# qdrant/qdrant

Measured on AMD Instinct MI355X. Metric: QPS @ recall@10, brute-force, d=768 10M vecs, f32 cosine top-10, higher is better.
Workload: dtype f32 (int8 prefilter + exact f32 re-score)

## Files before the change

### qdrant_amd/csrc/api_core.hip

```cpp
#include "api_internal.hpp"

namespace qmx {

static thread_local std::string g_last_error;
const std::string &last_error_text() { return g_last_error; }

void set_error(const char *fmt, ...) {
    char buf[1024];
    va_list ap;
    va_start(ap, fmt);
    vsnprintf(buf, sizeof(buf), fmt, ap);
    va_end(ap);
    g_last_error = buf;
}

int32_t hip_status(hipError_t e, const char *what, const char *file, int line) {
    set_error("HIP error %d (%s) at %s:%d: %s", (int)e, hipGetErrorString(e), file, line, what);
    (void)hipGetLastError();
    switch (e) {
        case hipErrorOutOfMemory: return QMX_ERR_OUT_OF_MEMORY;
        case hipErrorNoDevice:
        case hipErrorInvalidDevice:
        case hipErrorNoBinaryForGpu:
        case hipErrorInsufficientDriver: return QMX_ERR_NO_DEVICE;
        case hipErrorNotReady: return QMX_ERR_NOT_READY;
        case hipErrorInvalidValue: return QMX_ERR_BAD_ARG;
        default: return QMX_ERR_OTHER;
    }
}

static const char *const g_option_names[OPT_COUNT] = {"no_mfma_scan", "no_mfma16", "no_prescan", "prescan_shift", "hnsw_log_cap", "no_split_scan", "split_min_queries", "no_split256", "no_pq_pair", "no_pq_prefilter", "pq_prefilter_min_queries", "hnsw_pq_per_cu", "tq_rotate_block", "no_topk_small", "verify_max_per_query", "hnsw_pq_direct_walk", "hnsw_pq_table_build", "hnsw_no_pq_prefilter", "hnsw_no_lds_visited", "pq_lut_no_lds", "hnsw_per_cu", "hnsw_reference_heap_order", "tq_wide_min_queries", "tq_wide_high_digit", "sq_wide_min_queries", "i8_resident", "debug"};
struct OptionTable {
    std::atomic<int64_t> v[OPT_COUNT];
    int64_t initial[OPT_COUNT];
    OptionTable() {
        for (int i = 0; i < OPT_COUNT; ++i) {
            char env[64] = "QMX_";
            size_t k = 4;
            for (const char *c = g_option_names[i]; *c && k + 1 < sizeof(env); ++c) env[k++] = (char)toupper((unsigned char)*c);
            env[k] = 0;
            const char *e = getenv(env);
            int64_t val = 0;
            if (e) { val = (*e >= '0' && *e <= '9') ? atoll(e) : 1; }
            if (i == OPT_PRESCAN_SHIFT && !e) val = 10;
            if (i == OPT_SPLIT_MIN_QUERIES && !e) val = 1;
            if (i == OPT_PQ_PREFILTER_MIN_QUERIES && !e) val = 4;
            if (i == OPT_TQ_WIDE_MIN_QUERIES && !e) val = 33;
            if (i == OPT_SQ_WIDE_MIN_QUERIES && !e) val = 33;
            if (i == OPT_I8_RESIDENT && !e) val = 1;
            initial[i] = val;
            v[i].store(val, std::memory_order_relaxed);
        }
    }
};
static OptionTable g_options;
int64_t option(Option o) { return g_options.v[o].load(std::memory_order_relaxed); }

static thread_local const void *g_last_kernel = nullptr;
const void *last_noted_kernel() { return g_last_kernel; }
void note_kernel(const void *host_function) { g_last_kernel = host_function; }

void clear_stale_error() {
    hipError_t e = hipGetLastError();
    if (e != hipSuccess) {
// ... 98 lines not shown
```

### qdrant_amd/csrc/api_search.hip

```cpp
#include "api_internal.hpp"

extern "C" {



static int32_t split_stage(qmx_query *q, const char *what) {
    if (option(OPT_DEBUG) < 2) return QMX_OK;
    hipError_t e = hipStreamSynchronize(q->stream);
    fprintf(stderr, "[qmx] split stage %-28s %s\n", what, e == hipSuccess ? "ok" : hipGetErrorString(e));
    fflush(stderr);
    return e == hipSuccess ? QMX_OK : QMX_ERR_OTHER;
}

static int32_t verify_pool(qmx_query *q, unsigned char *plan, VerifyPool *vp) {
    const uint32_t cap = (uint32_t)std::min<uint64_t>(std::max<uint64_t>((uint64_t)q->nq * SPLIT_VCAP, 262144), 1u << 26);
    QMX_TRY(q->sp_ver.reserve(((size_t)cap * 2 + (size_t)q->nq * 2) * 4));
    QMX_TRY(q->sp_vscores.reserve((size_t)cap * 4));
    uint32_t *b = (uint32_t *)q->sp_ver.p;
    vp->ids = b;
    vp->qsel = b + cap;
    vp->off = b + (size_t)2 * cap;
    vp->cnt = vp->off + q->nq;
    vp->used = (uint32_t *)(plan + 24);
    vp->cap = cap;
// ... 334 lines not shown
            QMX_TRY(q->sp_probe.reserve((size_t)q->nq * (split_i8_probe() + 1) * 4));
            QMX_TRY(q->sp_pscores.reserve((size_t)q->nq * split_i8_probe() * 4));
        }
        plan = (unsigned char *)q->sp_plan.p;
        float *f = (float *)q->sp_f32.p;
        sp_qnorm = f; sp_thr = f + 256; sp_band = f + 512; sp_scales = f + 768; sp_qmax = f + 1024;
        const int sshift = (int)std::min<int64_t>(std::max<int64_t>(option(OPT_PRESCAN_SHIFT) + (s->d_rows_split ? 1 : -2), 1), 20);
        const uint64_t S = std::min<uint64_t>(n_cand, std::max<uint64_t>(n_cand >> sshift, 8192));
        if (q->sp_sample_n != S || q->sp_sample_of != n_cand) {
            QMX_TRY(q->sp_sample.reserve((size_t)S * 4));
            ::qmx::clear_stale_error();
            hipLaunchKernelGGL(sample_ids_kernel, dim3((uint32_t)((S + 255) / 256)), dim3(256), 0, q->stream, (uint32_t *)q->sp_sample.p, (uint32_t)S, n_cand / S);
            QMX_HIP(hipGetLastError());
            q->sp_sample_n = S;
            q->sp_sample_of = n_cand;
        }
        QMX_HIP(hipMemsetAsync(plan, 0, pl.zero_bytes, q->stream));
    }
    for (uint32_t tile0 = 0; tile0 < q->nq; tile0 += TQ) {
        const uint32_t nq_tile = std::min<uint32_t>(TQ, q->nq - tile0);
        if (split && (nq_tile > MAX_QT_TOPK || s->d_rows_split)) {
            if (is_stopped && *is_stopped) {
                set_error("search cancelled");
                return QMX_ERR_CANCELLED;
            }
            const uint32_t S = (uint32_t)q->sp_sample_n;
            const uint32_t *d_sample = (const uint32_t *)q->sp_sample.p;
            uint64_t *gthr = (uint64_t *)q->gthr.p + tile0;
            ScanArgs a;
            fill_args(q, tile0, nq_tile, a);
            a.n_cand = n_cand;
            a.top = top;
            QMX_TRY(q->scores.reserve((size_t)nq_tile * S * sizeof(float)));
            QMX_TRY(score_matrix_enqueue(q, tile0, nq_tile, d_sample, S, (float *)q->scores.p, S, nullptr));
            QMX_TRY(launch_custom_topk(q->stream, (const float *)q->scores.p, S, d_sample, a.del, nq_tile, top, d_out + (size_t)tile0 * top, d_counts + tile0, gthr));
            QMX_TRY(split_stage(q, "prescan"));
            if (s->split_i8) {
                float *sp_texact = sp_qnorm, *sp_qscale = sp_qmax;
                QMX_TRY(launch_split_i8_pack(q->stream, (const float *)q->enc.p + (size_t)tile0 * s->dim, nq_tile, s->dim, s->d_i8_scale, gthr, s->d_i8_stats,
                                             s->row_norm_max, q->sp_bq.p, sp_qscale, sp_band, sp_thr, sp_texact, (uint32_t *)q->sp_cnt.p, SPLIT_QT_MAX));
                QMX_TRY(split_stage(q, "int8 pack"));
                const uint32_t np = split_i8_probe();
                uint32_t *probe_ids = (uint32_t *)q->sp_probe.p, *probe_cnt = probe_ids + (size_t)q->nq * np;
                int *tile_ovf = (int *)(plan + pl.tile_ovf) + split_tiles.size();
                const uint32_t sstride = 16;
                for (uint32_t ph = 1; ph <= 2; ++ph) {
                    const uint32_t phase = ph | (sstride << 8);
                    size_t slot = 0;
                    if (timed) QMX_TRY(timing_begin(q, &slot));
                    QMX_TRY(launch_scan_i8copy(q->stream, a, q->sp_bq.p, sp_qscale, sp_thr, s->num_cus, s->d_rows_split, q->sp_wl.p, phase));
                    q->last_kernel = last_noted_kernel();
                    if (timed) QMX_TRY(timing_end(q, slot));
                    QMX_TRY(launch_split_regroup(q->stream, a, q->sp_wl.p, s->num_cus, (uint64_t *)q->sp_cand.p, (uint32_t *)q->sp_cnt.p, SPLIT_CAND_CAP, tile_ovf,
                                                 phase, SPLIT_QT));
                    QMX_TRY(launch_split_i8_probe(q->stream, (const uint64_t *)q->sp_cand.p, (const uint32_t *)q->sp_cnt.p, SPLIT_CAND_CAP, sp_band, nq_tile, top, tile_ovf,
                                                  probe_ids + (size_t)tile0 * np, probe_cnt + tile0));
                    const void *scan_kernel = q->last_kernel;
                    PairSel psel{nullptr, np, probe_cnt};
                    QMX_TRY(score_pairs_device(q, psel, probe_ids, (uint64_t)(tile0 + nq_tile) * np, (float *)q->sp_pscores.p, false));
                    q->last_kernel = scan_kernel;
                    QMX_TRY(launch_split_i8_bound(q->stream, (const float *)q->sp_pscores.p + (size_t)tile0 * np, probe_cnt + tile0, nq_tile, top, sp_band, sp_qscale,
                                                  sp_thr, sp_texact));
                }
                QMX_TRY(split_stage(q, "int8 scan"));
                QMX_TRY(launch_split_select(q->stream, (const uint64_t *)q->sp_cand.p, (const uint32_t *)q->sp_cnt.p, SPLIT_CAND_CAP, sp_band, nq_tile, top, vp, tile0,
                                            tile_ovf, (uint32_t *)(plan + pl.ovf_q) + tile0, (SplitStats *)plan, sp_texact));
                QMX_TRY(split_stage(q, "select"));
                split_tiles.push_back({tile0, nq_tile});
// ... 363 lines not shown
```

### qdrant_amd/csrc/common.hpp

```cpp
#pragma once
#include <hip/hip_runtime.h>
#include <hip/hip_fp16.h>
#include <stdint.h>
#include <atomic>
#include <string>

#include "../../include/qdrant_amd.h"

namespace qmx {

void set_error(const char *fmt, ...);
int32_t hip_status(hipError_t e, const char *what, const char *file, int line);
void clear_stale_error();

enum Option {
    OPT_NO_MFMA_SCAN = 0,
    OPT_NO_MFMA16,
    OPT_NO_PRESCAN,
    OPT_PRESCAN_SHIFT,
    OPT_HNSW_LOG_CAP,
    OPT_NO_SPLIT_SCAN,
    OPT_SPLIT_MIN_QUERIES,
    OPT_NO_SPLIT256,
    OPT_NO_PQ_PAIR,
    OPT_NO_PQ_PREFILTER,
    OPT_PQ_PREFILTER_MIN_QUERIES,
    OPT_HNSW_PQ_PER_CU,
    OPT_TQ_ROTATE_BLOCK,
    OPT_NO_TOPK_SMALL,
    OPT_VERIFY_MAX_PER_QUERY,
    OPT_HNSW_PQ_DIRECT_WALK,
    OPT_HNSW_PQ_TABLE_BUILD,
    OPT_HNSW_NO_PQ_PREFILTER,
    OPT_HNSW_NO_LDS_VISITED,
    OPT_PQ_LUT_NO_LDS,
    OPT_HNSW_PER_CU,
    OPT_HNSW_REFERENCE_HEAP_ORDER,
    OPT_TQ_WIDE_MIN_QUERIES,
    OPT_TQ_WIDE_HIGH_DIGIT,
    OPT_SQ_WIDE_MIN_QUERIES,
    OPT_I8_RESIDENT,
    OPT_DEBUG,
    OPT_COUNT
};
int64_t option(Option o);
struct DeviceOnce {
    std::atomic<uint64_t> done{0};
    int dev = 0;
    bool need() {
        if (hipGetDevice(&dev) != hipSuccess) { dev = 0; return true; }
        return dev >= 64 || !(done.load(std::memory_order_acquire) & (1ull << dev));
    }
    void mark() { if (dev < 64) done.fetch_or(1ull << dev, std::memory_order_release); }
};
void note_kernel(const void *host_function);
#define QMX_NOTE_KERNEL(fn) ::qmx::note_kernel(reinterpret_cast<const void *>(fn))

#define QMX_HIP(expr)                                                        \
    do {                                                                     \
        hipError_t e__ = (expr);                                             \
        if (e__ != hipSuccess) return ::qmx::hip_status(e__, #expr, __FILE__, __LINE__); \
    } while (0)

#define QMX_TRY(expr)                           \
    do {                                        \
        int32_t s__ = (expr);                   \
        if (s__ != QMX_OK) return s__;          \
    } while (0)

#define QMX_REQUIRE(cond, code, ...)            \
    do {                                        \
        if (!(cond)) {                          \
            ::qmx::set_error(__VA_ARGS__);      \
            return (code);                      \
// ... 89 lines not shown
```

### qdrant_amd/csrc/custom_query.hip

```cpp
#include "custom_combine.hpp"
#include "kernels.hpp"

namespace qmx {

__device__ __forceinline__ float custom_combine(const qmx_custom_query &q, const float *sims, uint64_t stride, const float *coefs) {
    const float *s = sims + (uint64_t)q.first * stride;
    return custom_score_by(q.kind, q.n_a, q.n_b, coefs + q.coef_first, [&](uint32_t e) { return s[(uint64_t)e * stride]; });
}

__global__ __launch_bounds__(256) void custom_combine_kernel(const qmx_custom_query *queries, uint32_t n_queries, const float *sims, uint64_t n,
                                                             const float *coefs, float *out) {
    const uint64_t c = (uint64_t)blockIdx.x * 256 + threadIdx.x;
    const uint32_t qi = blockIdx.y;
    if (c >= n || qi >= n_queries) return;
    out[(uint64_t)qi * n + c] = custom_combine(queries[qi], sims + c, n, coefs);
}

int32_t launch_custom_combine(hipStream_t st, const qmx_custom_query *d_queries, uint32_t n_queries, const float *d_sims, uint64_t n,
                              const float *d_coefs, float *d_out) {
    if (n == 0 || n_queries == 0) return QMX_OK;
    ::qmx::clear_stale_error();
    hipLaunchKernelGGL(custom_combine_kernel, dim3((uint32_t)((n + 255) / 256), n_queries), dim3(256), 0, st, d_queries, n_queries, d_sims, n, d_coefs, d_out);
    QMX_HIP(hipGetLastError());
    return QMX_OK;
// ... 201 lines not shown
            if (k != 0 && k >= t) surv[atomicAdd(&sh_cnt, 1u)] = k;
        }
        __syncthreads();
        const uint32_t cnt = sh_cnt;
        for (uint32_t i = threadIdx.x; i < cnt; i += CT_BLOCK) {
            const uint64_t my = surv[i];
            uint32_t r = 0;
            for (uint32_t j = 0; j < cnt; ++j) r += (surv[j] > my || (surv[j] == my && j < i)) ? 1u : 0u;
            if (r < ptop) {
                qmx_scored_point p;
                p.idx = key_idx(my);
                p.score = key_score(my);
                out[(uint64_t)q * top + off + r] = p;
                if (r == ptop - 1) sh_bound = my;
            }
        }
        const uint32_t found = cnt < ptop ? cnt : ptop;
        for (uint32_t i = found + threadIdx.x; i < ptop; i += CT_BLOCK) out[(uint64_t)q * top + off + i] = qmx_scored_point{0u, 0.0f};
        total += found;
        __syncthreads();
        bound = sh_bound;
        if (bound == 0) {
            for (uint32_t i = off + WAVE + threadIdx.x; i < top; i += CT_BLOCK) out[(uint64_t)q * top + i] = qmx_scored_point{0u, 0.0f};
            break;
        }
        __syncthreads();
    }
    if (threadIdx.x == 0) {
        out_counts[q] = total;
        if (bound_out) bound_out[q] = total == top ? bound : 0ull;
    }
}

int32_t launch_custom_topk(hipStream_t st, const float *d_scores, uint64_t n, const uint32_t *d_ids, const DeletedView &del, uint32_t n_queries,
                           uint32_t top, qmx_scored_point *d_out, uint32_t *d_counts, uint64_t *d_bound) {
    if (n_queries == 0) return QMX_OK;
    ::qmx::clear_stale_error();
    if (n >= 1 && n <= CTS_MAX_N && !option(OPT_NO_TOPK_SMALL)) {
        static thread_local DeviceOnce attr_once;
        if (attr_once.need()) {
            QMX_HIP(hipFuncSetAttribute(reinterpret_cast<const void *>(custom_topk_small_kernel), hipFuncAttributeMaxDynamicSharedMemorySize, (int)(CTS_MAX_N * 8)));
            attr_once.mark();
        }
        hipLaunchKernelGGL(custom_topk_small_kernel, dim3(n_queries), dim3(CT_BLOCK), (size_t)n * 8, st, d_scores, (uint32_t)n, d_ids, del, top, d_out, d_counts, d_bound);
        QMX_HIP(hipGetLastError());
        return QMX_OK;
    }
    hipLaunchKernelGGL(custom_topk_kernel, dim3(n_queries), dim3(CT_BLOCK), 0, st, d_scores, n, d_ids, del, top, d_out, d_counts, d_bound);
    QMX_HIP(hipGetLastError());
    return QMX_OK;
}

}
```

### qdrant_amd/csrc/kernels.hpp

```cpp
#pragma once
#include "common.hpp"

namespace qmx {

constexpr int MAX_QT = 16;
constexpr int SCAN_BLOCK = 512;
constexpr int MAX_TOP_FAST = 64;

struct TqEc {
    const int16_t *weights;
    const float *xm;
    float weight_scale, mm_const;
};
struct ScanArgs {
    const void *rows;
    uint64_t n_rows;
    uint64_t row_stride;
    uint32_t dim;
    uint32_t nseg;
    uint32_t rem_pieces;
    uint32_t tail_start;
    uint32_t aux_off;
    uint32_t nq;
    const void *queries;
// ... 186 lines not shown
    uint32_t *vis_log;
    uint32_t log_cap;
    uint32_t *sel_ids;
    float *sel_scores;
    uint32_t *sel_cnt;
    uint32_t *lock;
    uint32_t lds_query_bytes;
    uint32_t row_bytes;
    const unsigned char *batch_queries;
    uint64_t batch_q_stride;
    uint32_t *next;
};
int32_t launch_hnsw_build_bq(hipStream_t st, const ScanArgs &a, const HnswBuildArgs &h, int phase, uint32_t grid, int *per_cu);
int32_t launch_hnsw_build_sq(hipStream_t st, int distance, const ScanArgs &a, const HnswBuildArgs &h, int phase, uint32_t grid, int *per_cu);
int32_t launch_hnsw_build_dense(hipStream_t st, int dtype, int distance, const ScanArgs &a, const HnswBuildArgs &h, int phase,
                                uint32_t grid, int *per_cu);
int32_t launch_hnsw_build_maxsim_dense(hipStream_t st, int dtype, int distance, const ScanArgs &a, const HnswBuildArgs &h, int phase, uint32_t grid,
                                       int *per_cu);
int32_t launch_hnsw_build_maxsim_sq(hipStream_t st, int distance, const ScanArgs &a, const HnswBuildArgs &h, int phase, uint32_t grid, int *per_cu);
int32_t launch_hnsw_build_maxsim_bq(hipStream_t st, const ScanArgs &a, const HnswBuildArgs &h, int phase, uint32_t grid, int *per_cu);
int32_t launch_hnsw_build_tq(hipStream_t st, const ScanArgs &a, const HnswBuildArgs &h, int phase, uint32_t grid, int *per_cu);
int32_t launch_hnsw_build_tq_l1(hipStream_t st, const ScanArgs &a, const HnswBuildArgs &h, int phase, uint32_t grid, int *per_cu, uint32_t rot_dim,
                                uint32_t padded_dim);
int32_t launch_hnsw_build_pq(hipStream_t st, const ScanArgs &a, const HnswBuildArgs &h, int phase, uint32_t grid, int *per_cu);
int32_t launch_hnsw_build_maxsim_pq(hipStream_t st, const ScanArgs &a, const HnswBuildArgs &h, int phase, uint32_t grid, int *per_cu);
int32_t launch_hnsw_build_maxsim_tq(hipStream_t st, const ScanArgs &a, const HnswBuildArgs &h, int phase, uint32_t grid, int *per_cu);
int32_t launch_pq_pair_table(hipStream_t st, uint32_t distance, uint32_t dim, const qmx_pq_params &pq, const float *d_centroids, float *d_pair);
int32_t launch_u8_row_norms(hipStream_t st, const void *rows, uint64_t row_stride, uint64_t n, uint32_t dim, uint32_t flags, float *norms_f, int32_t *norms_i);
constexpr uint32_t HNSW_LDS_QUERY_MAX = 150 * 1024;

int32_t launch_scan_dense(hipStream_t st, int dtype, int distance, int qt, ScanMode mode,
                          const ScanArgs &a, int num_cus, uint32_t *grid_out);
int32_t launch_scan_f32_mfma(hipStream_t st, int qt, ScanMode mode, const ScanArgs &a, int num_cus, uint32_t *grid_out);
bool sq_mfma_ok(uint32_t distance, uint32_t actual_dim);
int32_t launch_scan_sq_mfma(hipStream_t st, int qt, ScanMode mode, const ScanArgs &a, int num_cus, uint32_t *grid_out);
int32_t launch_scan_f16_mfma(hipStream_t st, int qt, ScanMode mode, const ScanArgs &a, int num_cus, uint32_t *grid_out);
struct PairSel {
    const uint32_t *qsel;
    uint32_t per_query;
    const uint32_t *counts;
    const uint32_t *limit;
    __device__ __forceinline__ uint32_t query_of(uint64_t item) const {
        if (qsel) return qsel[item];
        if (per_query) return (uint32_t)(item / per_query);
        return (uint32_t)item;
    }
    __device__ __forceinline__ bool live(uint64_t item, uint32_t qi) const {
        if (limit && item >= (uint64_t)*limit) return false;
        if (per_query && counts) return (uint32_t)(item % per_query) < counts[qi];
        return true;
    }
};

int32_t launch_pairs_dense(hipStream_t st, int dtype, int distance, const ScanArgs &a, const PairSel &sel,
                           uint64_t n_items, int num_cus);
int32_t launch_pairs_sq(hipStream_t st, int distance, const ScanArgs &a, const PairSel &sel, uint64_t n_items, int num_cus);
int32_t launch_scan_sq(hipStream_t st, int distance, int qt, ScanMode mode, const ScanArgs &a, int num_cus,
                       uint32_t *grid_out);
int32_t launch_sq_encode(hipStream_t st, int distance, const qmx_sq_params &sp, uint32_t dim, const float *in, uint64_t n,
                         uint8_t *codes_out, uint64_t codes_stride, float *offsets_out, uint8_t *rows_out, int is_query,
                         uint32_t aux_off);
int32_t launch_sq_split(hipStream_t st, const void *rows, uint64_t row_stride, uint64_t n, uint32_t actual_dim, void *codes,
                        float *offsets);
int32_t launch_sq_gather_rows(hipStream_t st, const void *codes, const float *offsets, uint32_t actual_dim, const uint32_t *ids,
                              uint32_t n, uint64_t n_rows, void *rows_out, int *err_flag);
int32_t launch_sq_internal_query(hipStream_t st, const void *codes, const float *offsets, uint32_t actual_dim, const uint32_t *ids,
// ... 19 lines not shown
size_t pq_prefilter_table_bytes(uint32_t m, uint32_t nq);
uint32_t pq_prefilter_grid(int num_cus, uint32_t nq, uint32_t *n_slabs_out);
size_t pq_prefilter_wlists_counts_bytes(uint32_t grid);
size_t pq_prefilter_wlists_bytes(uint32_t grid, uint32_t wcap);
int32_t launch_pq_lut8(hipStream_t st, const void *d_luts, uint32_t q_stride, uint32_t nq, uint32_t m, uint32_t ncent, const uint64_t *d_gthr, void *d_table8,
                       int32_t *d_thr, float *d_band);
int32_t launch_pq_prefilter(hipStream_t st, const ScanArgs &a, const void *d_rot, const void *d_table8, const int32_t *d_thr, uint32_t nq, int num_cus,
                            void *d_wlists, uint32_t wcap, uint32_t *grid_out);
int32_t launch_split_refine(hipStream_t st, const uint64_t *d_cand, const uint32_t *d_cand_cnt, uint32_t cap, const float *d_band, uint32_t nq, uint32_t top,
                            const float *d_scales, float *d_thr);
size_t split_wlists_bytes(int num_cus);
int32_t launch_split_regroup(hipStream_t st, const ScanArgs &a, const void *d_wlists, int num_cus, uint64_t *d_cand, uint32_t *d_cand_cnt, uint32_t cap,
                             int *d_overflow, uint32_t phase, uint32_t qt);
size_t split_copy_bytes(uint64_t n, uint32_t dim, int half);
int32_t launch_split_copy(hipStream_t st, const void *rows, uint64_t row_stride, uint64_t n, uint32_t dim, float row_scale, void *d_out, int half);
struct SplitStats {
    unsigned long long candidates;
    unsigned long long verified;
    uint32_t fallback_queries;
    uint32_t pad;
};
struct VerifyPool {
    uint32_t *ids, *qsel, *off, *cnt, *used;
    uint32_t cap;
    uint32_t max_per_query;
};
int32_t launch_split_select(hipStream_t st, const uint64_t *d_cand, const uint32_t *d_cand_cnt, uint32_t cap, const float *d_band, uint32_t nq, uint32_t top,
                            const VerifyPool &pool, uint32_t q_base, const int *d_tile_overflow, uint32_t *d_ovf_q, SplitStats *d_stats,
                            const float *d_t_exact = nullptr, bool tighten = false);
bool split_i8_dim_ok(uint32_t dim);
size_t split_i8_copy_bytes(uint64_t n, uint32_t dim);
size_t split_i8_query_bytes(uint32_t dim);
uint32_t split_i8_probe();
int32_t launch_split_i8_colstats(hipStream_t st, const void *rows, uint64_t row_stride, uint64_t n, uint32_t dim, uint32_t *d_colmax, float *d_colsq);
float split_i8_choose_scales(const float *colmax, const float *colsq, uint64_t n, uint32_t dim, float *scale);
int32_t launch_split_i8_rowstats(hipStream_t st, const void *rows, uint64_t row_stride, uint64_t n, uint32_t dim, const float *d_scale, uint32_t *d_stats);
int32_t launch_split_i8_copy(hipStream_t st, const void *rows, uint64_t row_stride, uint64_t n, uint32_t dim, const float *d_scale, void *d_out);
int32_t launch_split_i8_pack(hipStream_t st, const float *d_q, uint32_t nq, uint32_t dim, const float *d_scale, const uint64_t *d_gthr, const uint32_t *d_row_stats,
                             float row_norm_max, void *d_bq, float *d_qscale, float *d_band, float *d_thr, float *d_t_exact, uint32_t *d_cand_cnt, uint32_t n_cnt);
int32_t launch_scan_i8copy(hipStream_t st, const ScanArgs &a, const void *d_bq, const float *d_qscale, const float *d_thr, int num_cus, const void *d_rows_i8,
                           void *d_wlists, uint32_t phase);
int32_t launch_split_i8_probe(hipStream_t st, const uint64_t *d_cand, const uint32_t *d_cand_cnt, uint32_t cap, const float *d_band, uint32_t nq, uint32_t top,
                              const int *d_tile_overflow, uint32_t *d_probe_ids, uint32_t *d_probe_cnt);
int32_t launch_split_i8_bound(hipStream_t st, const float *d_scores, uint32_t *d_probe_cnt, uint32_t nq, uint32_t top, const float *d_band, const float *d_qscale,
                              float *d_thr, float *d_t_exact);
bool tq4w_shape_ok(const ScanArgs &a);
size_t tq4w_query_bytes(uint32_t code_bytes);
size_t tq4w_wlists_counts_bytes(int num_cus);
size_t tq4w_wlists_bytes(int num_cus);
uint32_t tq4w_wcap();
int32_t launch_tq4w_stats(hipStream_t st, const float *d_sf, const float *d_l2, const void *d_rows, uint64_t row_stride, uint32_t code_bytes, uint64_t n, uint32_t *d_stats);
int32_t launch_tq4w_pack(hipStream_t st, const ScanArgs &a, const uint64_t *d_gthr, float sf_min, float sf_max, float l2_min, float l2_max, uint32_t c1, int high_only,
                         void *d_bq, int32_t *d_thr_i,
                         float *d_qinfo, float *d_band, uint32_t *d_cand_cnt, uint32_t n_cnt);
int32_t launch_scan_tq4w(hipStream_t st, const ScanArgs &a, const void *d_bq, const int32_t *d_thr_i, const float *d_qinfo, const float *d_band_high_only, int num_cus,
                         void *d_wlists, uint32_t *grid_out);
bool sqw_shape_ok(const ScanArgs &a);
size_t sqw_query_bytes(uint32_t dim);
size_t sqw_wlists_counts_bytes(int num_cus);
size_t sqw_wlists_bytes(int num_cus);
uint32_t sqw_wcap();
int32_t launch_sqw_stats(hipStream_t st, const float *d_off, uint64_t n, float multiplier, int32_t *d_bi, uint32_t *d_stats);
int32_t launch_sqw_pack(hipStream_t st, const ScanArgs &a, const uint64_t *d_gthr, float off_absmax, void *d_bq, int32_t *d_thr_i, float *d_qinfo, float *d_band,
                        uint32_t *d_cand_cnt, uint32_t n_cnt);
int32_t launch_scan_sqw(hipStream_t st, const ScanArgs &a, const void *d_bq, const int32_t *d_thr_i, const int32_t *d_bi, const float *d_qinfo, int num_cus,
                        void *d_wlists, uint32_t *grid_out);
// ... 12 lines not shown
int32_t launch_bq_encode(hipStream_t st, const float *d_in, uint64_t n, uint32_t dim, uint32_t encoding, const float *d_mean, const float *d_stddev,
                         uint8_t *d_out, uint64_t out_stride);
int32_t launch_scan_pq(hipStream_t st, ScanMode mode, const ScanArgs &a, int num_cus, uint32_t *grid_out);
int32_t launch_pairs_pq(hipStream_t st, const ScanArgs &a, const PairSel &sel, uint64_t n_items, int num_cus);
int32_t launch_pq_lut(hipStream_t st, uint32_t distance, uint32_t dim, const qmx_pq_params &pq, const float *d_centroids,
                      const float *d_queries, uint32_t nq, float *d_lut);
int32_t launch_pq_internal(hipStream_t st, uint32_t distance, uint32_t dim, const qmx_pq_params &pq, const float *d_centroids,
                           const float *d_pair, const void *rows, uint64_t row_stride, uint64_t n_rows, const uint32_t *a_ids, const uint32_t *b_ids,
                           uint32_t n, float *out, int *err_flag);
int32_t launch_pq_train(hipStream_t st, uint32_t dim, uint32_t chunk_size, uint32_t n_centroids, const float *d_data, uint64_t n,
                        uint32_t max_iters, float accuracy, uint32_t threads, float *d_centroids, uint32_t *iters_host);
int32_t launch_pq_encode(hipStream_t st, uint32_t dim, const qmx_pq_params &pq, const float *d_centroids, const float *d_in,
                         uint64_t n, uint8_t *d_codes);
int32_t launch_pack_queries(hipStream_t st, int dtype, int distance, const void *src, int src_is_encoded,
                            uint32_t src_stride, uint32_t nq, uint32_t dim, void *tile, uint32_t q_stride, uint32_t aux_off);
int32_t launch_merge_keys(hipStream_t st, const uint64_t *partial, uint32_t n_lists,
                          uint32_t qt_stride, uint32_t nq, uint32_t top, qmx_scored_point *out,
                          uint32_t *out_counts, uint32_t out_stride = 0, uint32_t out_offset = 0,
                          uint64_t *next_bound = nullptr, const int *run_if = nullptr, const uint32_t *out_map = nullptr, uint32_t shared_grid = 0);
int32_t launch_merge_points(hipStream_t st, const qmx_scored_point *lists, const uint32_t *list_counts,
                            const uint32_t *list_idx_base, uint32_t n_lists, uint32_t nq, uint32_t k, qmx_scored_point *out,
                            uint32_t *out_counts, uint64_t list_stride = 0, uint64_t count_stride = 0);
int32_t launch_split_candidates(hipStream_t st, const qmx_scored_point *cand, const uint32_t *cand_cnt, uint32_t n_per, uint32_t nq,
                                uint32_t *ids, uint32_t top, qmx_scored_point *out, uint32_t *out_counts);
int32_t launch_sort_scored(hipStream_t st, const float *scores, const uint32_t *ids, const uint32_t *counts, uint32_t n_per_query, uint32_t nq, uint32_t top,
                           qmx_scored_point *out, uint32_t *out_counts, const uint32_t *offsets = nullptr);

int32_t launch_custom_combine(hipStream_t st, const qmx_custom_query *d_queries, uint32_t n_queries, const float *d_sims, uint64_t n,
                              const float *d_coefs, float *d_out);
int32_t launch_maxsim(hipStream_t st, const float *d_sims, uint64_t n_rows, const uint32_t *d_qfirst, uint32_t n_queries, const uint64_t *d_offsets,
                      uint32_t n_points, const uint32_t *d_ids, uint64_t n, float *d_out, int *err_flag);
int32_t launch_custom_topk(hipStream_t st, const float *d_scores, uint64_t n, const uint32_t *d_ids, const DeletedView &del, uint32_t n_queries,
                           uint32_t top, qmx_scored_point *d_out, uint32_t *d_counts, uint64_t *d_bound = nullptr);

int32_t launch_cosine_preprocess_f32(hipStream_t st, const float *in, float *out, uint64_t n, uint32_t dim);
int32_t launch_cast_f32(hipStream_t st, int dst_dtype, const float *in, void *out, uint64_t count);
int32_t launch_minmax_f32(hipStream_t st, const float *in, uint64_t count, float *min_out, float *max_out);
int32_t launch_gather_rows(hipStream_t st, const void *rows, uint64_t row_stride, uint64_t row_bytes,
                           const uint32_t *ids, uint32_t n, uint64_t n_rows, void *out, int *err_flag);

struct SparseRows {
    const uint64_t *off;
    const uint32_t *idx;
    const float *val;
    uint64_t n;
};
struct SparseQueries {
    const uint64_t *off;
    const uint32_t *idx;
    const float *val;
};
struct SparsePlan {
    const uint32_t *off;
    const uint64_t *start;
    const uint64_t *end;
    const float *w;
};
uint32_t sparse_tile_ids();
uint32_t sparse_ids_lists(uint64_t n_ids);
int32_t launch_sparse_check_rows(hipStream_t st, const uint64_t *offsets, const uint32_t *idx, uint64_t n, uint32_t *flags);
int32_t launch_sparse_sort_rows(hipStream_t st, const uint64_t *offsets, uint32_t *idx, float *val, uint64_t n);
int32_t launch_sparse_remap(hipStream_t st, uint32_t *idx, uint64_t nnz, const uint32_t *keys, const uint32_t *vals, uint64_t m, uint32_t *missing);
int32_t sparse_build_postings(hipStream_t st, const uint64_t *offsets, const uint32_t *idx, const float *val, uint64_t n, uint64_t nnz, uint64_t *post,
                              uint32_t *dims, uint32_t *counts, uint32_t *n_dims_dev);
int32_t launch_sparse_score_matrix(hipStream_t st, const SparseRows &r, const SparseQueries &qs, uint32_t q0, uint32_t nq, const uint32_t *ids, uint64_t n,
                                   float *scores, uint64_t stride, int *err);
// ... 49 lines not shown
```

### qdrant_amd/csrc/scan_mfma.hip

```cpp
#include "scan_common.hpp"

namespace qmx {

typedef float f32x4 __attribute__((ext_vector_type(4)));


template <int XORMASK>
__device__ __forceinline__ float swz_xor(float v) {
    return __int_as_float(__builtin_amdgcn_ds_swizzle(__float_as_int(v), (XORMASK << 10) | 0x1F));
}
__device__ __forceinline__ float ror8(float v) {
    return __int_as_float(__builtin_amdgcn_update_dpp(0, __float_as_int(v), 0x128 , 0xF, 0xF, true));
}
__device__ __forceinline__ float swap16_add(float a, float b) {
    const auto r = __builtin_amdgcn_permlane16_swap(__float_as_uint(a), __float_as_uint(b), false, false);
    return __uint_as_float(r[0]) + __uint_as_float(r[1]);
}

template <int QW, int QSPLIT, int D, bool NT, int NWAVES, bool FAST, bool QH, bool HAS_IDS, int MODE>
__device__ __forceinline__ void scan_f32_mfma_body(const ScanArgs &a, unsigned char *smem) {
    constexpr int MF_BLOCK = NWAVES * 64, MF_NW = NWAVES;
    constexpr int GQ = QH ? 8 : 4;
    constexpr int TR = QH ? 4 : 8;
    constexpr int NG = QW / GQ;
// ... 286 lines not shown
    QMX_HIP(hipOccupancyMaxActiveBlocksPerMultiprocessor(&per_cu, kfn, MF_BLOCK, lds));
    if (per_cu < 1) per_cu = 1;
    const uint64_t n_tiles = (a.n_cand + (QH ? 3 : 7)) / (QH ? 4 : 8);
    const uint64_t want = (n_tiles + NSTREAM - 1) / NSTREAM;
    const uint64_t cap = (uint64_t)num_cus * per_cu;
    uint32_t grid = (uint32_t)(want < cap ? want : cap);
    if (grid < 1) grid = 1;
    if (grid_out) {
        if (*grid_out && MODE == SCAN_TOPK && grid > *grid_out) grid = *grid_out;
        *grid_out = grid;
    }
    uint32_t grid_y = 1;
    if (MODE == SCAN_SCORES && a.nq > (uint32_t)QT) {
        const uint32_t groups = (a.nq + QT - 1) / QT;
        if ((uint64_t)grid * groups <= cap) grid_y = groups;
    }
    ::qmx::clear_stale_error();
    QMX_NOTE_KERNEL(kfn);
    hipLaunchKernelGGL(kfn, dim3(grid, grid_y), dim3(MF_BLOCK), lds, st, a);
    QMX_HIP(hipGetLastError());
    return QMX_OK;
}

template <int QW, int QSPLIT, int D, bool NT, int NWAVES = 8, bool FAST = false, bool QH = false>
static int32_t launch_mfma_qt(hipStream_t st, ScanMode mode, const ScanArgs &a, int num_cus, uint32_t *grid) {
    const bool ids = a.ids != nullptr;
    if (mode == SCAN_TOPK)
        return ids ? launch_mfma_inst<QW, QSPLIT, D, NT, NWAVES, FAST, QH, true, SCAN_TOPK>(st, a, num_cus, grid)
                   : launch_mfma_inst<QW, QSPLIT, D, NT, NWAVES, FAST, QH, false, SCAN_TOPK>(st, a, num_cus, grid);
    return ids ? launch_mfma_inst<QW, QSPLIT, D, NT, NWAVES, FAST, QH, true, SCAN_SCORES>(st, a, num_cus, grid)
               : launch_mfma_inst<QW, QSPLIT, D, NT, NWAVES, FAST, QH, false, SCAN_SCORES>(st, a, num_cus, grid);
}

int32_t launch_scan_f32_mfma(hipStream_t st, int qt, ScanMode mode, const ScanArgs &a, int num_cus, uint32_t *grid_out) {
    switch (qt) {
        case 8: return launch_mfma_qt<8, 1, 4, true>(st, mode, a, num_cus, grid_out);
        case 16:
            if (mfma16_scan_ok(16, mode, a)) return launch_scan_f32_mfma16(st, 16, a, num_cus, grid_out);
            if (a.nseg % 12 == 0) return launch_mfma_qt<16, 1, 6, true, 8, true>(st, mode, a, num_cus, grid_out);
            return launch_mfma_qt<16, 1, 12, true>(st, mode, a, num_cus, grid_out);
        case 32: {
            if (mfma16_scan_ok(32, mode, a)) return launch_scan_f32_mfma16(st, 32, a, num_cus, grid_out);
#ifdef QMX_TUNING
            static const int variant = getenv("QMX_MFMA_VARIANT") ? atoi(getenv("QMX_MFMA_VARIANT")) : 0;
            if (variant == 1) return launch_mfma_qt<32, 1, 6, true, 8, false, true>(st, mode, a, num_cus, grid_out);
            if (variant == 2 && a.nseg % 12 == 0) return launch_mfma_qt<32, 1, 6, true, 8, true, true>(st, mode, a, num_cus, grid_out);
            if (variant == 3 && a.nseg % 24 == 0) return launch_mfma_qt<32, 1, 12, true, 8, true, true>(st, mode, a, num_cus, grid_out);
#endif
            if (a.nseg % 12 == 0) return launch_mfma_qt<16, 2, 6, true, 8, true>(st, mode, a, num_cus, grid_out);
            return launch_mfma_qt<16, 2, 12, true>(st, mode, a, num_cus, grid_out);
        }
    }
    if (qt == 64 && mfma16_scan_ok(64, mode, a)) return launch_scan_f32_mfma16(st, 64, a, num_cus, grid_out);
    set_error("unsupported MFMA query tile %d", qt);
    return QMX_ERR_BAD_ARG;
}

}
```

### qdrant_amd/csrc/scan_split.hip

```cpp
#include <type_traits>

#include "scan_common.hpp"

namespace qmx {

typedef _Float16 half8 __attribute__((ext_vector_type(8)));
typedef _Float16 half4 __attribute__((ext_vector_type(4)));
typedef float f32x4s __attribute__((ext_vector_type(4)));

constexpr int SP_BM = 256;
constexpr int SP_QT = 128;
constexpr int SP_QT_MAX = 256;
constexpr int SP_THREADS = 768;
constexpr int SP_CONSUMERS = 8;
constexpr int SP_A_UNITS = SP_BM * 2 * 4;
constexpr int SP_B_UNITS = SP_QT * 2 * 4;
constexpr int SP_BRING = 4;
constexpr int SP_LDS = (2 * SP_A_UNITS + SP_BRING * SP_B_UNITS) * 16;

__device__ __forceinline__ uint32_t sp_unit(uint32_t t, uint32_t hl, uint32_t kq, uint32_t m) { return ((t * 2 + hl) * 4 + kq) * 16 + (m ^ (2 * kq)); }

__device__ __forceinline__ void sp_split4(const f32x4s v, float scale, half4 &h, half4 &l) {
#pragma unroll
    for (int i = 0; i < 4; ++i) {
// ... 1725 lines not shown
        }
    }
    for (uint32_t i = 0; i < dim; ++i) {
        float f = (float)best[i];
        const float floor_s = colmax[i] > 1.0e-30f ? colmax[i] / 127.0f : 1.0f;
        scale[i] = f >= floor_s ? f : floor_s;
    }
    return best_g >= 1.0e29 ? 0.0f : (float)best_g;
}
int32_t launch_split_i8_rowstats(hipStream_t st, const void *rows, uint64_t row_stride, uint64_t n, uint32_t dim, const float *d_scale, uint32_t *d_stats) {
    QMX_REQUIRE(split_i8_dim_ok(dim), QMX_ERR_BAD_ARG, "int8 copy of dim %u", dim);
    ::qmx::clear_stale_error();
    QMX_HIP(hipMemsetAsync(d_stats, 0, 16, st));
    if (n) hipLaunchKernelGGL(sp_i8_row_stats_kernel, dim3(2048), dim3(256), 0, st, (const unsigned char *)rows, row_stride, n, dim, d_scale, d_stats);
    QMX_HIP(hipGetLastError());
    return QMX_OK;
}
int32_t launch_split_i8_copy(hipStream_t st, const void *rows, uint64_t row_stride, uint64_t n, uint32_t dim, const float *d_scale, void *d_out) {
    if (n == 0) return QMX_OK;
    ::qmx::clear_stale_error();
    hipLaunchKernelGGL(sp_i8_copy_kernel, dim3(8192), dim3(256), 0, st, (const unsigned char *)rows, row_stride, n, dim, d_scale, (uint4 *)d_out);
    QMX_HIP(hipGetLastError());
    return QMX_OK;
}
int32_t launch_split_i8_pack(hipStream_t st, const float *d_q, uint32_t nq, uint32_t dim, const float *d_scale, const uint64_t *d_gthr, const uint32_t *d_row_stats,
                             float row_norm_max, void *d_bq, float *d_qscale, float *d_band, float *d_thr, float *d_t_exact, uint32_t *d_cand_cnt, uint32_t n_cnt) {
    QMX_REQUIRE(nq <= (uint32_t)SP_QT, QMX_ERR_BAD_ARG, "int8 tile of %u queries", nq);
    ::qmx::clear_stale_error();
    hipLaunchKernelGGL(sp_i8_pack_kernel, dim3(SP_QT), dim3(256), (size_t)dim * 4, st, d_q, nq, dim, d_scale, d_gthr, d_row_stats, row_norm_max, (uint4 *)d_bq,
                       d_qscale, d_band, d_thr, d_t_exact, d_cand_cnt, n_cnt);
    QMX_HIP(hipGetLastError());
    return QMX_OK;
}
int32_t launch_scan_i8copy(hipStream_t st, const ScanArgs &a, const void *d_bq, const float *d_qscale, const float *d_thr, int num_cus, const void *d_rows_i8,
                           void *d_wlists, uint32_t phase) {
    const uint32_t nch_r = a.dim / 128;
    const bool resident = option(OPT_I8_RESIDENT) > 0 && nch_r <= SP8R_MAX_NCH;
    void (*kfn)(const ScanArgs, const SplitArgs) = resident ? scan_i8copy_kernel_res<1> : scan_i8copy_kernel;
    const size_t lds_bytes = resident ? sp8r_lds_bytes(nch_r) : (size_t)SP8_LDS;
    static thread_local DeviceOnce attr_once;
    if (attr_once.need()) {
        QMX_HIP(hipFuncSetAttribute(reinterpret_cast<const void *>(scan_i8copy_kernel), hipFuncAttributeMaxDynamicSharedMemorySize, SP8_LDS));
        QMX_HIP(hipFuncSetAttribute(reinterpret_cast<const void *>(scan_i8copy_kernel_res<1>), hipFuncAttributeMaxDynamicSharedMemorySize, (int)sp8r_lds_bytes(SP8R_MAX_NCH)));
        attr_once.mark();
    }
    QMX_REQUIRE(d_rows_i8 && d_wlists && split_i8_dim_ok(a.dim), QMX_ERR_BAD_ARG, "the int8 scan reads the int8 copy and writes per-wave candidate lists");
    SplitArgs s;
    s.rows_split = (const uint4 *)d_rows_i8;
    s.bq = (const uint4 *)d_bq;
    s.nchunks = a.dim / 128;
    s.nq = a.nq;
    s.row_scale = 1.0f;
    s.scales = d_qscale;
    s.thr = d_thr;
    s.cand = nullptr;
    s.cand_cnt = nullptr;
    s.cap = 0;
    s.wcap = SP_WCAP;
    s.wcnt = (uint32_t *)d_wlists;
    s.wlist = (uint4 *)((unsigned char *)d_wlists + split_wlists_counts_bytes(num_cus));
    s.phase = phase;
    const uint64_t n_tiles = split_phase_tiles((a.n_cand + SP3_BM - 1) / SP3_BM, phase);
    if (n_tiles == 0) return QMX_OK;
    const uint32_t grid = (uint32_t)std::max<uint64_t>(1, std::min<uint64_t>(n_tiles, (uint64_t)num_cus));
    ::qmx::clear_stale_error();
    QMX_NOTE_KERNEL(kfn);
// ... 21 lines not shown
```

Baseline: 98620.

## Score prescan sample with a small-LDS MFMA kernel and single-block sample top-k

For the int8 split path with f32 data, the prescan sample scoring now uses a reduced-footprint MFMA scan variant sized to fit in the LDS left over beside the resident int8 scan kernel. A new single-block-per-query radix-select top-k kernel replaces the generic top-k for small sample sizes. The aim is to cut prescan overhead and allow co-residency with the main scan. It adds an option to fall back and risks lower MFMA throughput from the narrower configuration.

```diff
diff --git a/qdrant_amd/csrc/api_core.hip b/qdrant_amd/csrc/api_core.hip
--- a/qdrant_amd/csrc/api_core.hip
+++ b/qdrant_amd/csrc/api_core.hip
@@ -29,7 +29,7 @@
     }
 }
 
-static const char *const g_option_names[OPT_COUNT] = {"no_mfma_scan", "no_mfma16", "no_prescan", "prescan_shift", "hnsw_log_cap", "no_split_scan", "split_min_queries", "no_split256", "no_pq_pair", "no_pq_prefilter", "pq_prefilter_min_queries", "hnsw_pq_per_cu", "tq_rotate_block", "no_topk_small", "verify_max_per_query", "hnsw_pq_direct_walk", "hnsw_pq_table_build", "hnsw_no_pq_prefilter", "hnsw_no_lds_visited", "pq_lut_no_lds", "hnsw_per_cu", "hnsw_reference_heap_order", "tq_wide_min_queries", "tq_wide_high_digit", "sq_wide_min_queries", "i8_resident", "debug"};
+static const char *const g_option_names[OPT_COUNT] = {"no_mfma_scan", "no_mfma16", "no_prescan", "prescan_shift", "hnsw_log_cap", "no_split_scan", "split_min_queries", "no_split256", "no_pq_pair", "no_pq_prefilter", "pq_prefilter_min_queries", "hnsw_pq_per_cu", "tq_rotate_block", "no_topk_small", "verify_max_per_query", "hnsw_pq_direct_walk", "hnsw_pq_table_build", "hnsw_no_pq_prefilter", "hnsw_no_lds_visited", "pq_lut_no_lds", "hnsw_per_cu", "hnsw_reference_heap_order", "tq_wide_min_queries", "tq_wide_high_digit", "sq_wide_min_queries", "i8_resident", "wide_sample_head", "debug"};
 struct OptionTable {
     std::atomic<int64_t> v[OPT_COUNT];
     int64_t initial[OPT_COUNT];
diff --git a/qdrant_amd/csrc/api_search.hip b/qdrant_amd/csrc/api_search.hip
--- a/qdrant_amd/csrc/api_search.hip
+++ b/qdrant_amd/csrc/api_search.hip
@@ -390,8 +390,23 @@
             a.n_cand = n_cand;
             a.top = top;
             QMX_TRY(q->scores.reserve((size_t)nq_tile * S * sizeof(float)));
-            QMX_TRY(score_matrix_enqueue(q, tile0, nq_tile, d_sample, S, (float *)q->scores.p, S, nullptr));
-            QMX_TRY(launch_custom_topk(q->stream, (const float *)q->scores.p, S, d_sample, a.del, nq_tile, top, d_out + (size_t)tile0 * top, d_counts + tile0, gthr));
+            bool beside = false;
+            if (s->split_i8 && s->dtype == QMX_DTYPE_F32 && mfma_scan_ok(s) && !option(OPT_WIDE_SAMPLE_HEAD)) {
+                ScanArgs pre;
+                fill_args(q, tile0, nq_tile, pre);
+                pre.ids = d_sample;
+                pre.n_cand = S;
+                pre.top = 1;
+                pre.scores = (float *)q->scores.p;
+                pre.scores_stride = S;
+                QMX_TRY(launch_scan_f32_mfma_beside(q->stream, pre, s->num_cus, split_i8_lds_beside(s->dim), &beside));
+            }
+            if (beside) {
+                QMX_TRY(launch_sample_topk(q->stream, (const float *)q->scores.p, S, d_sample, a.del, nq_tile, top, d_out + (size_t)tile0 * top, d_counts + tile0, gthr));
+            } else {
+                QMX_TRY(score_matrix_enqueue(q, tile0, nq_tile, d_sample, S, (float *)q->scores.p, S, nullptr));
+                QMX_TRY(launch_custom_topk(q->stream, (const float *)q->scores.p, S, d_sample, a.del, nq_tile, top, d_out + (size_t)tile0 * top, d_counts + tile0, gthr));
+            }
             QMX_TRY(split_stage(q, "prescan"));
             if (s->split_i8) {
                 float *sp_texact = sp_qnorm, *sp_qscale = sp_qmax;
diff --git a/qdrant_amd/csrc/common.hpp b/qdrant_amd/csrc/common.hpp
--- a/qdrant_amd/csrc/common.hpp
+++ b/qdrant_amd/csrc/common.hpp
@@ -40,6 +40,7 @@
     OPT_TQ_WIDE_HIGH_DIGIT,
     OPT_SQ_WIDE_MIN_QUERIES,
     OPT_I8_RESIDENT,
+    OPT_WIDE_SAMPLE_HEAD,
     OPT_DEBUG,
     OPT_COUNT
 };
diff --git a/qdrant_amd/csrc/custom_query.hip b/qdrant_amd/csrc/custom_query.hip
--- a/qdrant_amd/csrc/custom_query.hip
+++ b/qdrant_amd/csrc/custom_query.hip
@@ -257,6 +257,154 @@
     }
 }
 
+constexpr int STK_BLOCK = 256;
+constexpr int STK_E = 32;
+constexpr uint64_t STK_MAX_N = (uint64_t)STK_BLOCK * STK_E;
+constexpr uint32_t STK_SURV = 256;
+__global__ __launch_bounds__(STK_BLOCK) void sample_topk_kernel(const float *scores, uint32_t n, const uint32_t *ids, DeletedView del, uint32_t top,
+                                                                qmx_scored_point *out, uint32_t *out_counts, uint64_t *bound_out) {
+    constexpr int NW = STK_BLOCK / WAVE;
+    __shared__ uint64_t surv[STK_SURV];
+    __shared__ uint32_t hist[2][256];
+    __shared__ uint64_t sh_t[NW];
+    __shared__ uint64_t sh_bound;
+    __shared__ uint32_t sh_cnt;
+    const uint32_t q = blockIdx.x;
+    const int lane = threadIdx.x & 63, wave = threadIdx.x >> 6;
+    const float *row = scores + (uint64_t)q * n;
+    uint64_t kreg[STK_E];
+#pragma unroll
+    for (int e0 = 0; e0 < STK_E; e0 += 8) {
+        if ((uint32_t)e0 * STK_BLOCK >= n) {
+#pragma unroll
+            for (int u = 0; u < 8; ++u) kreg[e0 + u] = 0ull;
+            continue;
+        }
+        uint32_t id[8];
+        uint64_t key[8], keep[8];
+#pragma unroll
+        for (int u = 0; u < 8; ++u) {
+            const uint32_t c = (uint32_t)(e0 + u) * STK_BLOCK + threadIdx.x;
+            const uint32_t cc = c < n ? c : 0;
+            id[u] = ids ? ids[cc] : cc;
+            key[u] = c < n ? make_key(row[cc], id[u]) : 0ull;
+        }
+        live_masks<8>(del, id, keep);
+#pragma unroll
+        for (int u = 0; u < 8; ++u) kreg[e0 + u] = key[u] & keep[u];
+    }
+    hist[0][threadIdx.x] = 0;
+    uint32_t round = 0;
+    uint64_t bound = ~0ull;
+    uint32_t total = 0;
+    for (uint32_t off = 0; off < top; off += WAVE) {
+        const uint32_t ptop = top - off < (uint32_t)WAVE ? top - off : (uint32_t)WAVE;
+        uint64_t m = 0;
+#pragma unroll
+        for (int e = 0; e < STK_E; ++e) {
+            const uint64_t k = kreg[e] < bound ? kreg[e] : 0ull;
+            m = k > m ? k : m;
+        }
+        uint32_t rank = 0;
+        for (int j = 0; j < WAVE; ++j) rank += readlane_u64(m, j) > m ? 1u : 0u;
+        const uint64_t sel = __ballot(rank == ptop - 1 && m != 0);
+        const uint64_t tw = sel ? readlane_u64(m, __builtin_ctzll(sel)) : 0ull;
+        if (lane == 0) sh_t[wave] = tw;
+        if (threadIdx.x == 0) { sh_cnt = 0; sh_bound = 0; }
+        __syncthreads();
+        uint64_t t = 0;
+#pragma unroll
+        for (int w = 0; w < NW; ++w) t = sh_t[w] > t ? sh_t[w] : t;
+        uint64_t prefix = 0, hi_mask = 0;
+        uint32_t need = ptop;
+        bool enough = true;
+        for (int shift = 56; shift >= 0; shift -= 8, ++round) {
+            uint32_t *h = hist[round & 1];
+            if (shift != 56) __syncthreads();
+            hist[(round + 1) & 1][threadIdx.x] = 0;
+#pragma unroll
+            for (int e = 0; e < STK_E; ++e) {
+                const uint64_t k = kreg[e];
+                if (k < bound && k >= t && k != 0 && ((k ^ prefix) & hi_mask) == 0) atomicAdd(&h[(uint32_t)(k >> shift) & 255u], 1u);
+            }
+            __syncthreads();
+            uint32_t b[4];
+#pragma unroll
+            for (int i = 0; i < 4; ++i) b[i] = h[255 - 4 * lane - i];
+            const uint32_t tot = b[0] + b[1] + b[2] + b[3];
+            uint32_t incl = tot;
+#pragma unroll
+            for (int d = 1; d < WAVE; d <<= 1) {
+                const uint32_t up = (uint32_t)__shfl_up((int)incl, d, WAVE);
+                if (lane >= d) incl += up;
+            }
+            const uint32_t excl = incl - tot;
+            const uint64_t hit = __ballot(excl < need && need <= incl);
+            if (!hit) {
+                enough = false;
+                shift = -8;
+                continue;
+            }
+            uint32_t rem = need - excl, digit = 255u - 4u * (uint32_t)lane;
+#pragma unroll
+            for (int i = 0; i < 3; ++i)
+                if (rem > b[i] && digit == 255u - 4u * (uint32_t)lane - (uint32_t)i) { rem -= b[i]; --digit; }
+            const int src = __builtin_ctzll(hit);
+            digit = (uint32_t)__shfl((int)digit, src, WAVE);
+            need = (uint32_t)__shfl((int)rem, src, WAVE);
+            prefix |= (uint64_t)digit << shift;
+            hi_mask |= 0xFFull << shift;
+        }
+        const uint64_t kth = enough ? prefix : 0ull;
+#pragma unroll
+        for (int e = 0; e < STK_E; ++e) {
+            const uint64_t k = kreg[e];
+            if (k < bound && k >= t && k != 0 && k >= kth) {
+                const uint32_t slot = atomicAdd(&sh_cnt, 1u);
+                if (slot < STK_SURV) surv[slot] = k;
+            }
+        }
+        __syncthreads();
+        const uint32_t cnt = sh_cnt < STK_SURV ? sh_cnt : STK_SURV;
+        for (uint32_t i = threadIdx.x; i < cnt; i += STK_BLOCK) {
+            const uint64_t my = surv[i];
+            uint32_t r = 0;
+            for (uint32_t j = 0; j < cnt; ++j) r += (surv[j] > my || (surv[j] == my && j < i)) ? 1u : 0u;
+            if (r < ptop) {
+                qmx_scored_point p;
+                p.idx = key_idx(my);
+                p.score = key_score(my);
+                out[(uint64_t)q * top + off + r] = p;
+                if (r == ptop - 1) sh_bound = my;
+            }
+        }
+        const uint32_t found = cnt < ptop ? cnt : ptop;
+        for (uint32_t i = found + threadIdx.x; i < ptop; i += STK_BLOCK) out[(uint64_t)q * top + off + i] = qmx_scored_point{0u, 0.0f};
+        total += found;
+        __syncthreads();
+        bound = sh_bound;
+        if (bound == 0) {
+            for (uint32_t i = off + WAVE + threadIdx.x; i < top; i += STK_BLOCK) out[(uint64_t)q * top + i] = qmx_scored_point{0u, 0.0f};
+            break;
+        }
+        __syncthreads();
+    }
+    if (threadIdx.x == 0) {
+        out_counts[q] = total;
+        if (bound_out) bound_out[q] = total == top ? bound : 0ull;
+    }
+}
+
+int32_t launch_sample_topk(hipStream_t st, const float *d_scores, uint64_t n, const uint32_t *d_ids, const DeletedView &del, uint32_t n_queries,
+                           uint32_t top, qmx_scored_point *d_out, uint32_t *d_counts, uint64_t *d_bound) {
+    if (n < 1 || n > STK_MAX_N || option(OPT_WIDE_SAMPLE_HEAD) > 0) return launch_custom_topk(st, d_scores, n, d_ids, del, n_queries, top, d_out, d_counts, d_bound);
+    if (n_queries == 0) return QMX_OK;
+    ::qmx::clear_stale_error();
+    hipLaunchKernelGGL(sample_topk_kernel, dim3(n_queries), dim3(STK_BLOCK), 0, st, d_scores, (uint32_t)n, d_ids, del, top, d_out, d_counts, d_bound);
+    QMX_HIP(hipGetLastError());
+    return QMX_OK;
+}
+
 int32_t launch_custom_topk(hipStream_t st, const float *d_scores, uint64_t n, const uint32_t *d_ids, const DeletedView &del, uint32_t n_queries,
                            uint32_t top, qmx_scored_point *d_out, uint32_t *d_counts, uint64_t *d_bound) {
     if (n_queries == 0) return QMX_OK;
diff --git a/qdrant_amd/csrc/kernels.hpp b/qdrant_amd/csrc/kernels.hpp
--- a/qdrant_amd/csrc/kernels.hpp
+++ b/qdrant_amd/csrc/kernels.hpp
@@ -242,6 +242,7 @@
 int32_t launch_scan_dense(hipStream_t st, int dtype, int distance, int qt, ScanMode mode,
                           const ScanArgs &a, int num_cus, uint32_t *grid_out);
 int32_t launch_scan_f32_mfma(hipStream_t st, int qt, ScanMode mode, const ScanArgs &a, int num_cus, uint32_t *grid_out);
+int32_t launch_scan_f32_mfma_beside(hipStream_t st, const ScanArgs &a, int num_cus, size_t lds_budget, bool *taken);
 bool sq_mfma_ok(uint32_t distance, uint32_t actual_dim);
 int32_t launch_scan_sq_mfma(hipStream_t st, int qt, ScanMode mode, const ScanArgs &a, int num_cus, uint32_t *grid_out);
 int32_t launch_scan_f16_mfma(hipStream_t st, int qt, ScanMode mode, const ScanArgs &a, int num_cus, uint32_t *grid_out);
@@ -327,6 +328,7 @@
 size_t split_i8_copy_bytes(uint64_t n, uint32_t dim);
 size_t split_i8_query_bytes(uint32_t dim);
 uint32_t split_i8_probe();
+size_t split_i8_lds_beside(uint32_t dim);
 int32_t launch_split_i8_colstats(hipStream_t st, const void *rows, uint64_t row_stride, uint64_t n, uint32_t dim, uint32_t *d_colmax, float *d_colsq);
 float split_i8_choose_scales(const float *colmax, const float *colsq, uint64_t n, uint32_t dim, float *scale);
 int32_t launch_split_i8_rowstats(hipStream_t st, const void *rows, uint64_t row_stride, uint64_t n, uint32_t dim, const float *d_scale, uint32_t *d_stats);
@@ -405,6 +407,8 @@
                       uint32_t n_points, const uint32_t *d_ids, uint64_t n, float *d_out, int *err_flag);
 int32_t launch_custom_topk(hipStream_t st, const float *d_scores, uint64_t n, const uint32_t *d_ids, const DeletedView &del, uint32_t n_queries,
                            uint32_t top, qmx_scored_point *d_out, uint32_t *d_counts, uint64_t *d_bound = nullptr);
+int32_t launch_sample_topk(hipStream_t st, const float *d_scores, uint64_t n, const uint32_t *d_ids, const DeletedView &del, uint32_t n_queries,
+                           uint32_t top, qmx_scored_point *d_out, uint32_t *d_counts, uint64_t *d_bound);
 
 int32_t launch_cosine_preprocess_f32(hipStream_t st, const float *in, float *out, uint64_t n, uint32_t dim);
 int32_t launch_cast_f32(hipStream_t st, int dst_dtype, const float *in, void *out, uint64_t count);
diff --git a/qdrant_amd/csrc/scan_mfma.hip b/qdrant_amd/csrc/scan_mfma.hip
--- a/qdrant_amd/csrc/scan_mfma.hip
+++ b/qdrant_amd/csrc/scan_mfma.hip
@@ -342,6 +342,14 @@
                : launch_mfma_inst<QW, QSPLIT, D, NT, NWAVES, FAST, QH, false, SCAN_SCORES>(st, a, num_cus, grid);
 }
 
+int32_t launch_scan_f32_mfma_beside(hipStream_t st, const ScanArgs &a, int num_cus, size_t lds_budget, bool *taken) {
+    *taken = (size_t)16 * a.q_stride + 256 + 15 <= lds_budget;
+    if (!*taken) return QMX_OK;
+    uint32_t grid = 0;
+    if (a.nseg % 12 == 0) return launch_mfma_qt<16, 1, 6, true, 4, true>(st, SCAN_SCORES, a, num_cus, &grid);
+    return launch_mfma_qt<16, 1, 4, true, 4>(st, SCAN_SCORES, a, num_cus, &grid);
+}
+
 int32_t launch_scan_f32_mfma(hipStream_t st, int qt, ScanMode mode, const ScanArgs &a, int num_cus, uint32_t *grid_out) {
     switch (qt) {
         case 8: return launch_mfma_qt<8, 1, 4, true>(st, mode, a, num_cus, grid_out);
diff --git a/qdrant_amd/csrc/scan_split.hip b/qdrant_amd/csrc/scan_split.hip
--- a/qdrant_amd/csrc/scan_split.hip
+++ b/qdrant_amd/csrc/scan_split.hip
@@ -1781,6 +1781,11 @@
     QMX_HIP(hipGetLastError());
     return QMX_OK;
 }
+size_t split_i8_lds_beside(uint32_t dim) {
+    const uint32_t nch_r = dim / 128;
+    const bool resident = option(OPT_I8_RESIDENT) > 0 && nch_r <= SP8R_MAX_NCH;
+    return (size_t)160 * 1024 - (resident ? sp8r_lds_bytes(nch_r) : (size_t)SP8_LDS);
+}
 int32_t launch_scan_i8copy(hipStream_t st, const ScanArgs &a, const void *d_bq, const float *d_qscale, const float *d_thr, int num_cus, const void *d_rows_i8,
                            void *d_wlists, uint32_t phase) {
     const uint32_t nch_r = a.dim / 128;
```

After: 98480, median of 2. No clear change (-0.1%).
